# Vigilans/GomokuAI

Measured on AMD Instinct MI355X. Metric: board-evals/s, higher is better.
Workload: dtype int32; 1 GPU; batched AC-automaton position eval (K1), 65536 random-opening boards per GPU, 15x15, inputs resident in HBM; boards_per_gpu=65536, parallelism=boards sharded by rank, no collective, launch=hipGraph replay of the K steps

## Files before the change

gomokuai_amd/csrc/eval_kernel.hip:

```cpp
#include <algorithm>
#include <cstdlib>
#include <vector>

#include "capi_common.h"

namespace {

constexpr int kBoardsPerBlock = 16;
constexpr int kGroupBoards = 16;
constexpr int kThreads = 64 * kBoardsPerBlock;
constexpr int kCells = 225;
constexpr int kQueueCap = 448;
constexpr int kMaxBlocksPerCu = 1;

constexpr int kScoreWords = 4 * kCells;
constexpr int kCntWords = 3 * kCells + 1;
constexpr int kZeroWords = kScoreWords + kCntWords;
constexpr int kLineWords = 96;
constexpr int kColBase = 20, kDiagBase = 36, kAntiBase = 65;
#ifndef GMK_K1_TOTALS_COPIES
#define GMK_K1_TOTALS_COPIES 8
#endif
constexpr int kTotalsCopies = GMK_K1_TOTALS_COPIES;
constexpr int kMiscWords = 48;
constexpr int kBoardWords = kZeroWords + kLineWords + kQueueCap + kMiscWords;
static_assert(kZeroWords % 4 == 0 && kBoardWords % 4 == 0, "16-byte alignment of the per-board blocks");
constexpr int kStaticTableWords = 128 + kLineWords + 512 + 1560 + 4;

__constant__ uint32_t c_lane_jobs[64 * 2];
__constant__ uint32_t c_line_init[kLineWords];
constexpr int kScanSteps = 19;

__device__ __forceinline__ int dir_stride(int dir) { return (0x0E100F01u >> (8 * dir)) & 0xFFu; }

__device__ __forceinline__ uint64_t line_symbols(uint32_t line_word, int len) {
    return 2ull | (static_cast<uint64_t>(line_word) << 2) | (0xAull << (2 * len + 2));
}

__device__ __forceinline__ const __attribute__((address_space(3))) uint32_t* lds_word(uint32_t byte_address) {
    return reinterpret_cast<const __attribute__((address_space(3))) uint32_t*>(static_cast<uintptr_t>(byte_address));
}

__device__ __forceinline__ __attribute__((address_space(3))) uint32_t* lds_word_rw(uint32_t byte_address) {
    return reinterpret_cast<__attribute__((address_space(3))) uint32_t*>(static_cast<uintptr_t>(byte_address));
}

__device__ __forceinline__ uint32_t dfa_address(uint32_t table_word, uint32_t four) {
    uint32_t addr;
    asm("v_bfi_b32 %0, %1, %2, %3" : "=v"(addr) : "s"(0x3FF3u), "v"(table_word), "v"(four));
    return addr;
}

__device__ __forceinline__ uint32_t mul24(uint32_t a, uint32_t b) {
    uint32_t r;
    asm("v_mul_u32_u24 %0, %1, %2" : "=v"(r) : "v"(a), "s"(b));
    return r;
}

__device__ __forceinline__ void wave_phase_fence() {
    __builtin_amdgcn_fence(__ATOMIC_RELEASE, "wavefront");
    __builtin_amdgcn_wave_barrier();
    __builtin_amdgcn_fence(__ATOMIC_ACQUIRE, "wavefront");
}

__device__ __forceinline__ void deposit_match(uint32_t w0, uint32_t w1, int cell_at, int dir, int back_step,
                                              uint32_t* s_scores, uint32_t* s_cnt, uint32_t* s_misc, uint32_t* totals ) {
    const int type = w0 & 15, fav = (w0 >> 4) & 1;
    if (type == 8) { atomicOr(&s_misc[1], fav ? 1u : 2u); return; }
    atomicAdd(&totals[type], fav ? 0x10000u : 1u);
    const int endcell = cell_at + static_cast<int>((w0 >> 27) & 1u) * back_step;
    const uint32_t score = dir >= 2 ? (w1 >> 16) : (w1 & 0xFFFFu);
    unsigned long long* pair = reinterpret_cast<unsigned long long*>(s_scores) + fav;
    const uint32_t lo_opp = fav ? score : 0u, hi_opp = fav ? 0u : score;
    const uint32_t tslot = 5u - static_cast<uint32_t>(type);
    const bool feeds = tslot < 3u;
    uint32_t* cnt = s_cnt + (feeds ? tslot : 0u) * kCells;
    const uint32_t one = 1u << (4 * (fav * 4 + dir));
    const int n_dep = (w0 >> 8) & 7;
#pragma unroll
    for (int d = 0; d < 4; ++d) {
        if (d >= n_dep) break;
        const uint32_t f = (w0 >> (11 + 4 * d)) & 15u;
        const int c = endcell + static_cast<int>(f & 7u) * back_step;
        const bool both = (f & 8u) != 0u;
        atomicAdd(&pair[2 * c], (static_cast<unsigned long long>(both ? score : hi_opp) << 32) | (both ? score : lo_opp));
        if (both && feeds) atomicAdd(&cnt[c], one);
    }
}

__device__ __forceinline__ int counter_match(uint32_t w0, int k, int want) {
    const int type = w0 & 15, len = (w0 >> 5) & 7;
    const int back = k - static_cast<int>((w0 >> 27) & 1u) - 6;
    if (!w0 || type != want || back < 0 || back >= len) return -1;
    const int n_dep = (w0 >> 8) & 7;
    bool on_q = false;
#pragma unroll
    for (int d = 0; d < 4; ++d) {
        const uint32_t f = (w0 >> (11 + 4 * d)) & 15u;
        on_q |= d < n_dep && f == (8u | static_cast<uint32_t>(back));
    }
    return on_q ? back : -1;
}

__device__ __forceinline__ void add_counter_cells(uint32_t w0, int back, int q, int stride, uint32_t* opp) {
    const int n_dep = (w0 >> 8) & 7, endcell = q + back * stride;
#pragma unroll
    for (int d = 0; d < 4; ++d) {
        const uint32_t f = (w0 >> (11 + 4 * d)) & 15u;
        if (d < n_dep && static_cast<int>(f & 7u) != back) atomicAdd(&opp[4 * (endcell - static_cast<int>(f & 7u) * stride)], 600u);
    }
}

[[maybe_unused]] constexpr int kDensTiles = 7;
__host__ __device__ constexpr int dens_kt_lo(int m) { return (((32 * m) / 15 - 3) < 0 ? 0 : (32 * m) / 15 - 3) / 2; }
__host__ __device__ constexpr int dens_kt_hi(int m) { return (((32 * m + 31) / 15 + 3) > 14 ? 14 : (32 * m + 31) / 15 + 3) / 2; }
constexpr int kWtabDy = 13, kWtabEntryWords = 4, kWtabKindWords = kWtabDy * 15 * kWtabEntryWords, kWtabWords = 2 * kWtabKindWords;
__host__ __device__ constexpr int block_weight(int dy, int dx) {
    constexpr int w[4][7] = {{1, 3, 4, 0, 4, 3, 1}, {0, 3, 5, 4, 5, 3, 0}, {0, 4, 3, 3, 3, 4, 0}, {2, 0, 0, 1, 0, 0, 2}};
    return w[dy < 0 ? -dy : dy][dx + 3];
}

typedef int v4i __attribute__((ext_vector_type(4)));
typedef int v16i __attribute__((ext_vector_type(16)));

template <int KIND, int M>
__device__ __forceinline__ void density_tile_pass(const uint32_t (&own_rows)[8], const uint32_t (&other_rows)[8], int n_boards, int first_board, int lane,
                                                  const v4i* __restrict__ s_wtab, int32_t* __restrict__ out_density,
                                                  const uint2* __restrict__ s_lut, int plane_stride) {
    constexpr int lo = dens_kt_lo(M), hi = dens_kt_hi(M), nk = hi - lo + 1;
    constexpr int y0 = (32 * M) / 15, y1 = (32 * M + 31) / 15;
    const int n = lane & 31, h = lane >> 5;
    uint32_t occ = 0;
#pragma unroll
    for (int y = y0; y <= y1; ++y) {
        const uint32_t both = own_rows[y / 2] | other_rows[y / 2];
        const uint32_t r = ((y & 1) ? both >> 16 : both) & 0x7FFFu;
        const int at = 15 * y - 32 * M;
        occ |= at >= 0 ? r << at : r >> -at;
    }
    const int cell = 32 * M + n, yo = (cell * 0x8889) >> 19, xo = cell - 15 * yo;
    const v4i* w = s_wtab + KIND * (kWtabKindWords / kWtabEntryWords) + (2 * lo + h - yo + 6) * 15 + xo;
    v16i acc = {0, 0, 0, 0, 0, 0, 0, 0, 0, 0, 0, 0, 0, 0, 0, 0};
#pragma unroll
    for (int k = 0; k < nk; ++k) {
        const uint32_t r = (own_rows[lo + k] >> (16 * h)) & 0x7FFFu;
        const uint2 b0 = s_lut[r & 255u], b1 = s_lut[r >> 8];
        const v4i stones = {static_cast<int>(b0.x), static_cast<int>(b0.y), static_cast<int>(b1.x), static_cast<int>(b1.y)};
        acc = __builtin_amdgcn_mfma_i32_32x32x32_i8(stones, w[30 * k], acc, 0, 0, 0);
    }
    const int n_live = n_boards - first_board;
    int32_t* out = out_density + static_cast<size_t>(first_board) * 4 * plane_stride + KIND * plane_stride + 32 * M + n + h * (2 * 4 * plane_stride);
#pragma unroll
    for (int i = 0; i < 16; i += 2) {
        const int b = 4 * (i / 4) + (i % 4) / 2;
        const uint32_t wd = static_cast<uint32_t>(__builtin_amdgcn_ds_bpermute(8 * b + 16 * h, static_cast<int>(occ)));
        const int neg = __builtin_amdgcn_sbfe(static_cast<int>(wd), n, 1);
        if (b + 2 * h < n_live && plane_stride > 0) {
            out[b * 4 * plane_stride + 1 * 2 * plane_stride] = acc[i] ^ neg;
            out[b * 4 * plane_stride + 0 * 2 * plane_stride] = acc[i + 1] ^ neg;
        }
    }
}

__device__ __forceinline__ void density_planes_out(const uint16_t* __restrict__ planes, int n_boards, int first_board, int lane,
                                                   const v4i* __restrict__ s_wtab, int32_t* __restrict__ out_density,
                                                   const uint2* __restrict__ s_lut, int plane_stride) {
    const int n = lane & 31, plane = n & 1, board = first_board + (n >> 1);
    uint32_t own[8], other[8];
    {
        const uint4* p = reinterpret_cast<const uint4*>(planes + static_cast<size_t>(board < n_boards ? board : first_board) * 32);
        const uint4 a0 = p[plane * 2], a1 = p[plane * 2 + 1], b0 = p[2 - plane * 2], b1 = p[3 - plane * 2];
        own[0] = a0.x; own[1] = a0.y; own[2] = a0.z; own[3] = a0.w; own[4] = a1.x; own[5] = a1.y; own[6] = a1.z; own[7] = a1.w;
        other[0] = b0.x; other[1] = b0.y; other[2] = b0.z; other[3] = b0.w; other[4] = b1.x; other[5] = b1.y; other[6] = b1.z; other[7] = b1.w;
    }
    if ((lane >> 5) == 0 && board < n_boards && plane_stride > 0) {
        uint32_t c224 = 0, w224 = 0;
#pragma unroll
        for (int dy = -3; dy <= 0; ++dy) {
            const int y = 14 + dy;
            const uint32_t r = (y & 1) ? own[y >> 1] >> 16 : own[y >> 1] & 0xFFFFu;
#pragma unroll
            for (int dx = -3; dx <= 0; ++dx) {
                if (block_weight(dy, dx) == 0) continue;
                const uint32_t bit = (r >> (14 + dx)) & 1u;
                c224 += bit;
                w224 += bit * static_cast<uint32_t>(block_weight(dy, dx));
            }
        }
        const uint32_t neg = 0u - (((own[7] | other[7]) >> 14) & 1u);
        int32_t* out = out_density + static_cast<size_t>(board) * 4 * plane_stride + (1 - plane) * 2 * plane_stride;
        out[224] = static_cast<int32_t>(c224 ^ neg);
        out[plane_stride + 224] = static_cast<int32_t>(w224 ^ neg);
    }
#define GMK_PASS(K, M) density_tile_pass<K, M>(own, other, n_boards, first_board, lane, s_wtab, out_density, s_lut, plane_stride); __builtin_amdgcn_sched_barrier(0);
    GMK_PASS(0, 0) GMK_PASS(1, 0) GMK_PASS(0, 1) GMK_PASS(1, 1) GMK_PASS(0, 2) GMK_PASS(1, 2) GMK_PASS(0, 3) GMK_PASS(1, 3)
    GMK_PASS(0, 4) GMK_PASS(1, 4) GMK_PASS(0, 5) GMK_PASS(1, 5) GMK_PASS(0, 6) GMK_PASS(1, 6)
#undef GMK_PASS
}

__global__ __launch_bounds__(kThreads)
void eval_positions_kernel(const uint16_t* __restrict__ planes, int n_boards, int n_groups,
                           int32_t* __restrict__ out_scores, int32_t* __restrict__ out_density,
                           uint32_t* __restrict__ out_totals, int32_t* __restrict__ out_status,
                           const uint32_t* __restrict__ g_trans, const uint32_t* __restrict__ g_records,
                           int trans_words, int record_words, const uint32_t* __restrict__ g_wtab,
                           int phase_mask_arg, unsigned long long* __restrict__ prof) {
#ifdef GMK_PROFILE
    const int phase_mask = phase_mask_arg;
    unsigned long long t_acc[12] = {0, 0, 0, 0, 0, 0, 0, 0, 0, 0, 0, 0}, t_prev = __builtin_amdgcn_s_memtime();
#define GMK_STAMP(k) do { if (prof) { const unsigned long long t_now_ = __builtin_amdgcn_s_memtime(); t_acc[k] += t_now_ - t_prev; t_prev = t_now_; } } while (0)
#else
    constexpr int phase_mask = 0x7F;
    (void)phase_mask_arg; (void)prof;
#define GMK_STAMP(k) do { } while (0)
#endif
    extern __shared__ __attribute__((aligned(16))) uint32_t lds[];
    const uint4* s_rec = reinterpret_cast<const uint4*>(lds + trans_words);
    uint32_t* s_jobs = lds + trans_words + record_words;

    for (int i = threadIdx.x; i < trans_words; i += kThreads) lds[i] = g_trans[i];
    for (int i = threadIdx.x; i < record_words; i += kThreads) lds[trans_words + i] = g_records[i];
    if (threadIdx.x < 128) s_jobs[threadIdx.x] = c_lane_jobs[threadIdx.x];
    uint32_t* s_pads = s_jobs + 128;
    if (threadIdx.x < kLineWords) s_pads[threadIdx.x] = ~c_line_init[threadIdx.x] & 0xAAAAAAAAu;
    uint2* s_lut = reinterpret_cast<uint2*>(s_jobs + 128 + kLineWords);
    if (threadIdx.x < 256) s_lut[threadIdx.x] = make_uint2(((threadIdx.x & 15u) * 0x204081u) & 0x01010101u, ((threadIdx.x >> 4) * 0x204081u) & 0x01010101u);
    uint32_t* s_wtab_words = s_jobs + 128 + kLineWords + 512;
    for (int i = threadIdx.x; i < kWtabWords; i += kThreads) s_wtab_words[i] = g_wtab[i];
    const v4i* s_wtab = reinterpret_cast<const v4i*>(s_wtab_words);
    uint32_t* s_handout = s_wtab_words + kWtabWords;
    if (threadIdx.x < 4) s_handout[threadIdx.x] = threadIdx.x == 0 ? 2u * kBoardsPerBlock : 0u;

    const int wave = __builtin_amdgcn_readfirstlane(threadIdx.x >> 6), lane0 = threadIdx.x & 63;
    uint32_t* s_scores = lds + trans_words + record_words + kStaticTableWords + wave * kBoardWords;
    uint32_t* s_cnt = s_scores + kScoreWords;
    uint32_t* s_lines = s_scores + kZeroWords;
    uint32_t* s_queue = s_lines + kLineWords;
    uint32_t* s_misc = s_queue + kQueueCap;
#ifndef GMK_K1_TOTALS_HOT
    uint32_t* const my_totals = s_queue + kQueueCap - 8 * kTotalsCopies + (lane0 & (kTotalsCopies - 1)) * 8;
#else
    uint32_t* const my_totals = s_misc + 4;
#endif

    GMK_STAMP(0);

    const bool planes_out = out_density != nullptr && (phase_mask & 64) && !(phase_mask & 1024);
    int lane = lane0;
    const uint32_t job_a = c_lane_jobs[lane * 2], job_b = c_lane_jobs[lane * 2 + 1];
    const uint32_t line_init_lo = c_line_init[lane], line_init_hi = c_line_init[min(64 + lane, kLineWords - 1)];
    auto first_bit = [](uint32_t job) -> uint32_t {
        const uint32_t dir = (job >> 5) & 3u, first = (job >> 12) & 255u, y0 = (first * 0x8889u) >> 19, x0 = first - 15u * y0;
        return dir == 2u ? 2u * x0 : dir == 3u ? 2u * y0 : 0u;
    };
    const uint32_t norm_a = first_bit(job_a), norm_b = first_bit(job_b);
    uint32_t* s_rows = s_misc + 16;
    uint32_t cell_row4 = 0, cell_col = 0;
    for (int pass = 0; pass < 4; ++pass) {
        const int c = min(64 * pass + lane, kCells - 1), y = (c * 0x8889) >> 19;
        cell_row4 |= static_cast<uint32_t>(4 * y) << (8 * pass);
        cell_col |= static_cast<uint32_t>(c - 15 * y) << (8 * pass);
    }
    const uint16_t* row_ptr = planes + (lane & 15);
    uint32_t next_black = 0, next_white = 0, cur_black = 0, cur_white = 0;
    auto fetch_row = [&](int b) {
        const uint16_t* p = row_ptr + static_cast<size_t>(min(b, n_boards - 1)) * 32;
        next_black = p[0];
        next_white = p[16];
    };
    auto take_row = [&](int b) -> uint32_t { return lane < 16 && b < n_boards ? cur_black | (cur_white << 16) : 0u; };

    const int wg_g0 = static_cast<int>(static_cast<long long>(n_groups) * blockIdx.x / gridDim.x);
    const int wg_groups = static_cast<int>(static_cast<long long>(n_groups) * (blockIdx.x + 1) / gridDim.x) - wg_g0;
    const int wg_first = wg_g0 * kGroupBoards, wg_boards = min(wg_groups * kGroupBoards, n_boards - wg_first);
    auto hand_out = [&](int which) -> int {
        uint32_t v = 0;
        if (lane0 == 0) v = atomicAdd(&s_handout[which], 1u);
        return __builtin_amdgcn_readfirstlane(static_cast<int>(v));
    };
    int idx = wave, boards_done = 0;
    if (idx < wg_boards) fetch_row(wg_first + idx);
    asm volatile("" : "+v"(next_black), "+v"(next_white));
#pragma unroll 1
    for (;;) {
        const bool live = idx < wg_boards;
        const int board = wg_first + idx;
        cur_black = next_black; cur_white = next_white;
        int idx_next = idx;
        if (live) { idx_next = boards_done == 0 ? kBoardsPerBlock + wave : hand_out(0); fetch_row(wg_first + min(idx_next, wg_boards - 1)); }
        GMK_STAMP(11);

        if (live) {
            {
                uint4* z = reinterpret_cast<uint4*>(s_cnt) + lane;
    #pragma unroll
                for (int i = 0; i < kCntWords / 4; i += 64)
                    if (i + 64 <= kCntWords / 4 || lane < kCntWords / 4 - i) z[i] = make_uint4(0u, 0u, 0u, 0u);
            }
            s_lines[lane] = line_init_lo;
            if (lane < kLineWords - 64) s_lines[64 + lane] = line_init_hi;
            if (lane < kMiscWords) s_misc[lane] = 0;
#ifndef GMK_K1_TOTALS_HOT
            if (lane < 8 * kTotalsCopies) s_queue[kQueueCap - 8 * kTotalsCopies + lane] = 0;
#endif
            const uint32_t my_row = take_row(board);
            wave_phase_fence();
            {
                uint32_t cnt = static_cast<uint32_t>(__popc(my_row & 0x7FFFu)) | (static_cast<uint32_t>(__popc(my_row >> 16)) << 16);
                cnt += static_cast<uint32_t>(__builtin_amdgcn_update_dpp(0, static_cast<int>(cnt), 0x118, 0xF, 0xF, false));
                cnt += static_cast<uint32_t>(__builtin_amdgcn_update_dpp(0, static_cast<int>(cnt), 0x114, 0xF, 0xF, false));
                cnt += static_cast<uint32_t>(__builtin_amdgcn_update_dpp(0, static_cast<int>(cnt), 0x112, 0xF, 0xF, false));
                cnt += static_cast<uint32_t>(__builtin_amdgcn_update_dpp(0, static_cast<int>(cnt), 0x111, 0xF, 0xF, false));
                if (lane == 15) s_misc[0] = cnt;
            }
            {
                const uint32_t r = my_row;
                const uint32_t l1 = (r & 0x3FFF3FFFu) << 1, l2 = (r & 0x1FFF1FFFu) << 2, l3 = (r & 0x0FFF0FFFu) << 3;
                const uint32_t r1 = (r & 0x7FFE7FFEu) >> 1, r2 = (r & 0x7FFC7FFCu) >> 2, r3 = (r & 0x7FF87FF8u) >> 3;
                const int far = static_cast<int>(r | l3 | r3), near = static_cast<int>(r | l1 | l2 | r1 | r2);
                uint32_t g = l1 | l2 | l3 | r1 | r2 | r3;
                g |= static_cast<uint32_t>(__builtin_amdgcn_update_dpp(0, near, 0x111, 0xF, 0xF, true)) | static_cast<uint32_t>(__builtin_amdgcn_update_dpp(0, near, 0x101, 0xF, 0xF, true));
                g |= static_cast<uint32_t>(__builtin_amdgcn_update_dpp(0, near, 0x112, 0xF, 0xF, true)) | static_cast<uint32_t>(__builtin_amdgcn_update_dpp(0, near, 0x102, 0xF, 0xF, true));
                g |= static_cast<uint32_t>(__builtin_amdgcn_update_dpp(0, far, 0x113, 0xF, 0xF, true)) | static_cast<uint32_t>(__builtin_amdgcn_update_dpp(0, far, 0x103, 0xF, 0xF, true));
                const uint32_t empty = ~(r | (r >> 16)) & 0x7FFFu;
                if (lane < 15) s_rows[3 + lane] = r;
                const int gate = static_cast<int>(g & (empty | (empty << 16)));
    #pragma unroll
                for (int pass = 0; pass < 4; ++pass) {
                    const uint32_t gw = static_cast<uint32_t>(__builtin_amdgcn_ds_bpermute(static_cast<int>((cell_row4 >> (8 * pass)) & 0xFFu), gate)) >> ((cell_col >> (8 * pass)) & 0xFFu);
                    if (pass < 3 || lane < kCells - 192)
                        reinterpret_cast<uint4*>(s_scores)[64 * pass + lane] = make_uint4(((gw >> 16) & 1u) * 160u, 0u, 0u, (gw & 1u) * 160u);
                }
            }
            {
                const int y = lane >> 2, part = lane & 3;
                const uint32_t row = __shfl(my_row, min(y, 14));
                uint32_t row_sym = 0;
                for (uint32_t m = lane < 60 ? (row | (row >> 16)) & (0xFu << (4 * part)) & 0x7FFFu : 0u; m; m &= m - 1u) {
                    const int x = __ffs(m) - 1;
                    const uint32_t code = ((row >> x) & 1u) ? 3u : 2u;
                    const uint32_t at_x = code << (2 * x), at_y = code << (2 * y);
                    row_sym |= at_x;
                    atomicXor(&s_lines[kColBase + x], at_y);
                    atomicXor(&s_lines[kDiagBase + x - y + 14], at_x);
                    atomicXor(&s_lines[kAntiBase + x + y], at_y);
                }
                if (row_sym) atomicXor(&s_lines[y], row_sym);
            }
            wave_phase_fence();
            GMK_STAMP(1);
        }
        if (boards_done == 0) __syncthreads();
        if (live) {
            int n_queued = 0;
            if (phase_mask & 2) {
                const int len_a = static_cast<int>(job_a & 31u) - 3, len_b = static_cast<int>(job_b & 31u) - 3;
                uint64_t syms = line_symbols(s_lines[(job_a >> 20) & 127u] >> norm_a, len_a);
                syms |= line_symbols(s_lines[(job_b >> 20) & 127u] >> norm_b, len_b) << (2 * len_a + 6);
                syms |= 0xAAAAAAAAAAAAAAAAull << (2 * (len_a + len_b) + 12);
                const uint32_t cur = static_cast<uint32_t>(syms) << 2;
                const uint32_t rest = static_cast<uint32_t>(syms >> 28);
                uint32_t tw = 0;
                const uint32_t q_base = static_cast<uint32_t>(s_queue - lds) * 4u;
                const uint32_t q_full = q_base + 4u * (kQueueCap - 64);
                uint32_t q_at = q_base;
                auto push = [&](uint32_t word, int step) {
                    const bool emits = word > 0x1FFFFu;
                    const unsigned long long emitters = __ballot(emits);
                    if (emitters) {
                        if (emits) {
                            const uint32_t ahead = __builtin_amdgcn_mbcnt_hi(static_cast<uint32_t>(emitters >> 32), __builtin_amdgcn_mbcnt_lo(static_cast<uint32_t>(emitters), 0u));
                            *lds_word_rw(q_at + 4u * ahead) = (word & ~0x1FFFFu) | (static_cast<uint32_t>(lane) | static_cast<uint32_t>(step) << 6);
                        }
                        q_at = min(q_at + 4u * static_cast<uint32_t>(__popcll(emitters)), q_full);
                    }
                };
#pragma unroll
                for (int step = 0; step < kScanSteps; ++step) {
                    const uint32_t four = step < 15 ? __builtin_amdgcn_ubfe(cur, 2 * step, 4) : __builtin_amdgcn_ubfe(rest, 2 * (step - 15), 4);
                    const uint32_t addr = dfa_address(tw, four);
                    const uint32_t before = tw;
                    tw = *lds_word(addr);
                    if (step > 0) push(before, step - 1);
                }
                push(tw, kScanSteps - 1);
                n_queued = static_cast<int>((q_at - q_base) >> 2);
                if (q_at >= q_full) s_misc[2] = 1;
            }
            wave_phase_fence();
            GMK_STAMP(2);

            if (phase_mask & 4) {
                uint32_t qe_next = s_queue[min(lane, kQueueCap - 1)];
                for (int m = lane; m < n_queued; m += 64) {
                    const uint32_t qe = qe_next;
                    qe_next = s_queue[min(m + 64, kQueueCap - 1)];
                    const int src_lane = qe & 63, src_step = (qe >> 6) & 31;
                    const uint4 rec_now = s_rec[qe >> 17];
                    const uint32_t ja_now = s_jobs[src_lane * 2], jb_now = s_jobs[src_lane * 2 + 1];
                    const int seg_a = ja_now & 31u;
                    const bool second = src_step >= seg_a;
                    const uint32_t job = second ? jb_now : ja_now;
                    const int pos = src_step - 1 - (second ? seg_a : 0);
                    const int dir = (job >> 5) & 3, stride = (job >> 7) & 31;
                    const int cell_at = static_cast<int>((job >> 12) & 255u) + pos * stride;
                    deposit_match(rec_now.x, rec_now.y, cell_at, dir, -stride, s_scores, s_cnt, s_misc, my_totals);
                    if (rec_now.z) deposit_match(rec_now.z, rec_now.w, cell_at, dir, -stride, s_scores, s_cnt, s_misc, my_totals);
                }
            }
            wave_phase_fence();
#ifndef GMK_K1_TOTALS_HOT
            if (lane < 8) {
                const uint32_t* t = s_queue + kQueueCap - 8 * kTotalsCopies + lane;
                uint32_t sum = 0;
#pragma unroll
                for (int c = 0; c < kTotalsCopies; ++c) sum += t[8 * c];
                s_misc[4 + lane] = sum;
            }
#endif
            GMK_STAMP(3);

            int n_cand = 0;
            if (phase_mask & 8) {
                uint32_t any_cnt[4];
    #pragma unroll
                for (int pass = 0; pass < 4; ++pass) {
                    const int qc = min(64 * pass + lane, kCells - 1);
                    any_cnt[pass] = s_cnt[qc] | s_cnt[kCells + qc] | s_cnt[2 * kCells + qc];
                }
    #pragma unroll
                for (int pass = 0; pass < 4; ++pass) {
                    const int q = 64 * pass + lane;
                    const uint32_t any = any_cnt[pass];
                    const uint32_t upper = (any >> 1) | (any >> 2) | (any >> 3);
                    const uint32_t clipped = ((any | upper) & 0x11111111u) + (upper & 0x11111111u);
                    uint32_t cand = mul24(clipped, 0x1111u) & 0xE000u;
                    cand |= mul24(clipped >> 16, 0x11110u) & 0xE0000u;
                    if (pass == 3 && q >= kCells) cand = 0u;
                    const unsigned long long pushers = __ballot(cand != 0u);
                    if (pushers) {
                        if (cand) {
                            const int slot = n_cand + static_cast<int>(__builtin_amdgcn_mbcnt_hi(static_cast<uint32_t>(pushers >> 32),
                                                                       __builtin_amdgcn_mbcnt_lo(static_cast<uint32_t>(pushers), 0u)));
                            if (slot < kQueueCap / 2) s_queue[slot] = static_cast<uint32_t>(q) | cand;
                        }
                        n_cand += __popcll(pushers);
                    }
                }
            }
            wave_phase_fence();
            GMK_STAMP(4);

            if (n_cand > kQueueCap / 2) { s_misc[2] = 1; n_cand = kQueueCap / 2; }
            if (phase_mask & 2048) n_cand = 0;
            int n_comp_q = 0;
            if (phase_mask & 8)
            for (int v0 = 0; v0 < 2 * n_cand; v0 += 64) {
                const int v = v0 + lane;
                const int flag_shift = 13 + 4 * (v & 1);
                const uint32_t ce = s_queue[v >> 1];
                const int q = ce & 255, c = v & 1;
                bool queue = false;
                uint32_t ent1 = 0, ent2 = 0;
                if (v < 2 * n_cand && ((ce >> flag_shift) & 7u)) {
                    const uint32_t f3 = (s_cnt[q] >> (16 * c)) & 0xFFFFu, fd = (s_cnt[kCells + q] >> (16 * c)) & 0xFFFFu, f2 = (s_cnt[2 * kCells + q] >> (16 * c)) & 0xFFFFu;
                    uint32_t dens = 0;
                    const int qy = (q * 0x8889) >> 19, qx = q - 15 * qy;
                    {
                        const int half = c ? 0 : 16;
    #pragma unroll
                        for (int dy = -3; dy <= 3; ++dy) {
                            const uint32_t pattern = dy == 0 ? 0x77u : (dy == 3 || dy == -3) ? 0x49u : 0x3Eu;
                            const uint32_t mask = ((pattern << qx) >> 3) & 0x7FFFu;
                            dens += __popc((s_rows[3 + qy + dy] >> half) & mask);
                        }
                    }
                    if (dens >= 2u) {
                        const uint32_t up3 = (f3 >> 1) | (f3 >> 2) | (f3 >> 3), upd = (fd >> 1) | (fd >> 2) | (fd >> 3), up2 = (f2 >> 1) | (f2 >> 2) | (f2 >> 3);
                        const uint32_t sel3 = (f3 | up3) & 0x1111u;
                        const uint32_t seld = (fd | upd) & 0x1111u & ~sel3;
                        const uint32_t sel2 = (f2 | up2) & 0x1111u & ~(sel3 | seld);
                        const uint32_t strong = sel3 | seld, any_dir = strong | sel2;
                        const uint32_t twice_strong = (sel3 & up3) | (seld & upd), twice = twice_strong | (sel2 & up2);
                        const int n_comp = __popc(any_dir) + __popc(twice), threes = __popc(strong) + __popc(twice_strong);
                        if (n_comp < 2) {
                            s_misc[2] = 1;
                        } else {
                            const int ctype = min(threes, 2);
                            atomicAdd(&s_misc[12 + ctype], c ? 0x10000u : 1u);
                            const uint32_t crit = 600u * static_cast<uint32_t>(n_comp);
                            atomicAdd(reinterpret_cast<unsigned long long*>(s_scores) + 2 * q + c, (static_cast<unsigned long long>(crit) << 32) | crit);
                            queue = n_comp < 3 && !sel3;
                            const uint32_t b1 = static_cast<uint32_t>(__ffs(any_dir) - 1);
                            const uint32_t others = any_dir & (any_dir - 1u);
                            const uint32_t b2 = others ? static_cast<uint32_t>(__ffs(others) - 1) : b1;
                            const uint32_t ux = static_cast<uint32_t>(qx), uy = static_cast<uint32_t>(qy);
                            const uint32_t lines = (static_cast<uint32_t>(kColBase) << 8 | static_cast<uint32_t>(kDiagBase + 14) << 16 | static_cast<uint32_t>(kAntiBase) << 24)
                                                   + ((ux << 8) * 0x10101u) + uy * 0xFF0001u;
                            const uint32_t slots = ux * 0x0101u + uy * 0x1010u;
                            const uint32_t head = static_cast<uint32_t>(q) | (static_cast<uint32_t>(c) << 8);
                            auto entry = [&](uint32_t b) {
                                const uint32_t tslot = ((seld >> b) & 1u) ? 1u : 2u;
                                return head | (b >> 2) << 9 | tslot << 11 | __builtin_amdgcn_ubfe(lines, 2 * b, 8) << 13 | __builtin_amdgcn_ubfe(slots, b, 4) << 20;
                            };
                            ent1 = entry(b1);
                            ent2 = entry(b2);
                        }
                    }
                }
                const unsigned long long queuers = __ballot(queue);
                if (queue) {
                    const uint32_t slot = static_cast<uint32_t>(n_comp_q) + 2u * __builtin_amdgcn_mbcnt_hi(static_cast<uint32_t>(queuers >> 32),
                                                                                                          __builtin_amdgcn_mbcnt_lo(static_cast<uint32_t>(queuers), 0u));
                    if (slot < kQueueCap / 2) { s_queue[kQueueCap / 2 + slot] = ent1; s_queue[kQueueCap / 2 + slot + 1] = ent2; }
                    else s_misc[2] = 1;
                }
                n_comp_q += 2 * __popcll(queuers);
            }
            wave_phase_fence();
            GMK_STAMP(5);

            if (phase_mask & 16) {
                const int n_comp = min(n_comp_q, kQueueCap / 2);
                int lane_4 = lane;
                asm volatile("" : "+v"(lane_4));
                const int grp = lane_4 / 7, kk = lane_4 - 7 * grp, k = 6 + kk, start = k > 7 ? k - 7 : 0;
                for (int m0 = 0; m0 < n_comp; m0 += 9) {
                    const int m = m0 + grp;
                    const bool on = lane < 63 && m < n_comp;
                    const uint32_t ent = on ? s_queue[kQueueCap / 2 + m] : 0u;
                    const int q = ent & 255, c = (ent >> 8) & 1, dir = (ent >> 9) & 3, tslot = (ent >> 11) & 3;
                    const int stride = dir_stride(dir);
                    uint32_t hit_w0 = 0;
                    int hit_back = -1;
                    if (on) {
                        const uint32_t line = (ent >> 13) & 127u;
                        const uint32_t word = s_lines[line] | s_pads[line];
                        const int first = static_cast<int>((ent >> 20) & 15u) + start - 6;
                        const uint32_t cur = __builtin_amdgcn_alignbit(first >= 0 ? 0xAAAAAAAAu : word, first >= 0 ? word : 0xAAAAAAAAu,
                                                                       static_cast<uint32_t>(2 * first) & 31u) << 2;
                        uint32_t tw = 0;
    #pragma unroll
                        for (int i = 0; i < 8; ++i)
                            if (start + i <= k) tw = *lds_word(dfa_address(tw, __builtin_amdgcn_ubfe(cur, 2 * i, 4)));
                        if ((gmk::dev_trans_kinds(tw) >> tslot) & 1u) {
                            const uint4 rec = s_rec[gmk::dev_trans_record(tw)];
                            const int want = 5 - tslot;
                            hit_back = counter_match(rec.x, k, want);
                            hit_w0 = rec.x;
                            if (hit_back < 0) { hit_back = counter_match(rec.z, k, want); hit_w0 = rec.z; }
                        }
                    }
                    const unsigned long long hits = __ballot(hit_back >= 0);
                    const uint32_t mine = static_cast<uint32_t>(hits >> (7 * grp)) & 0x7Fu;
                    if (hit_back >= 0 && (mine & ((1u << kk) - 1u)) == 0u) add_counter_cells(hit_w0, hit_back, q, stride, s_scores + (c ? 2 : 1));
                }
            }
            wave_phase_fence();
            GMK_STAMP(6);

        }

        asm volatile("" : "+v"(next_black), "+v"(next_white));
        GMK_STAMP(7);

        if (planes_out && (!live || (boards_done & 15) == wave)) {
            for (;;) {
                const int burst = hand_out(1);
                if (burst >= wg_groups) break;
                int lane_p = lane0, first_p = (wg_g0 + burst) * kGroupBoards;
                asm volatile("" : "+v"(lane_p), "+s"(first_p));
                density_planes_out(planes, n_boards, first_p, lane_p, s_wtab, out_density, s_lut, (phase_mask & 512) ? 0 : (phase_mask & 256) ? 256 : kCells);
                GMK_STAMP(8);
                if (live) break;
            }
        }
        if (!live) break;
        if (live && (phase_mask & 32)) {
            int lane_b = lane;
            asm volatile("" : "+v"(lane_b));
            if (out_scores) {
                int32_t* dst = out_scores + static_cast<size_t>(board) * kScoreWords + lane_b;
                const int4* src = reinterpret_cast<const int4*>(s_scores);
                const int4 v0 = src[lane_b], v1 = src[lane_b + 64], v2 = src[lane_b + 128], v3 = src[min(lane_b + 192, kCells - 1)];
#ifdef GMK_K1_PLAIN_SCORES
#define GMK_STORE(p, v) (*(p) = (v))
#else
#define GMK_STORE(p, v) __builtin_nontemporal_store(v, p)
#endif
                const bool tail = lane_b + 192 < kCells;
                GMK_STORE(dst, v0.x); GMK_STORE(dst + 64, v1.x); GMK_STORE(dst + 128, v2.x); if (tail) GMK_STORE(dst + 192, v3.x);
                GMK_STORE(dst + kCells, v0.y); GMK_STORE(dst + kCells + 64, v1.y); GMK_STORE(dst + kCells + 128, v2.y); if (tail) GMK_STORE(dst + kCells + 192, v3.y);
                GMK_STORE(dst + 2 * kCells, v0.z); GMK_STORE(dst + 2 * kCells + 64, v1.z); GMK_STORE(dst + 2 * kCells + 128, v2.z); if (tail) GMK_STORE(dst + 2 * kCells + 192, v3.z);
                GMK_STORE(dst + 3 * kCells, v0.w); GMK_STORE(dst + 3 * kCells + 64, v1.w); GMK_STORE(dst + 3 * kCells + 128, v2.w); if (tail) GMK_STORE(dst + 3 * kCells + 192, v3.w);
#undef GMK_STORE
            }
            if (out_totals && lane_b < 11) out_totals[static_cast<size_t>(board) * 11 + lane_b] = s_misc[4 + lane_b];
            if (out_status && lane_b == 0) {
                const uint32_t wbits = s_misc[1], stones = s_misc[0];
                const int stones_b = stones & 0xFFFFu, stones_w = stones >> 16;
                const int winner = (wbits & 1u) ? 1 : (wbits & 2u) ? -1 : 0;
                const bool over = winner != 0 || stones_b + stones_w == kCells;
                const int to_move = over ? 0 : (stones_b == stones_w ? 1 : -1);
                out_status[board] = (over ? 1 : 0) | ((s_misc[2] || phase_mask != 0x7F) ? 2 : 0) | ((winner & 0xFF) << 8) | ((to_move & 0xFF) << 16);
            }
        }
        wave_phase_fence();
        GMK_STAMP(9);
        idx = idx_next; ++boards_done;
    }
#ifdef GMK_PROFILE
    if (prof && lane0 == 0) {
        for (int k = 0; k < 12; ++k) atomicAdd(&prof[k], t_acc[k]);
        atomicAdd(&prof[15], 1ull);
    }
#endif
#undef GMK_STAMP
}

struct LineJob { int len, x0, y0, dir; };

int upload_lane_jobs() {
    std::vector<LineJob> lines;
    for (int i = 0; i < 15; ++i) lines.push_back({15, 0, i, 0});
    for (int i = 0; i < 15; ++i) lines.push_back({15, i, 0, 1});
    for (int d = -10; d <= 10; ++d) lines.push_back({15 - std::abs(d), d > 0 ? d : 0, d > 0 ? 0 : -d, 2});
    for (int k = 4; k <= 24; ++k) { const int x0 = std::min(k, 14); lines.push_back({std::min(k, 28 - k) + 1, x0, k - x0, 3}); }
    std::stable_sort(lines.begin(), lines.end(), [](const LineJob& a, const LineJob& b) { return a.len > b.len; });
    uint32_t jobs[128];
    for (uint32_t& j : jobs) j = 3u | (15u << 20);
    auto pack = [](const LineJob& l) {
        const int line = l.dir == 0 ? l.y0 : l.dir == 1 ? kColBase + l.x0 : l.dir == 2 ? kDiagBase + l.x0 - l.y0 + 14 : kAntiBase + l.x0 + l.y0;
        const int stride = l.dir == 0 ? 1 : l.dir == 1 ? 15 : l.dir == 2 ? 16 : 14;
        return static_cast<uint32_t>((l.len + 3) | (l.dir << 5) | (stride << 7) | ((l.y0 * 15 + l.x0) << 12) | (line << 20));
    };
    int steps = 0;
    for (int lane = 0; lane < 64; ++lane) {
        jobs[lane * 2] = pack(lines[lane]);
        int total = lines[lane].len + 3;
        const int extra = 64 + (63 - lane);
        if (extra < static_cast<int>(lines.size())) { jobs[lane * 2 + 1] = pack(lines[extra]); total += lines[extra].len + 3; }
        steps = std::max(steps, total);
    }
    uint32_t init[kLineWords] = {};
    for (int i = 0; i < 15; ++i) init[i] = init[kColBase + i] = 0x3FFFFFFFu;
    for (int d = 0; d <= 28; ++d) init[kDiagBase + d] = init[kAntiBase + d] = ((1u << (2 * (15 - std::abs(d - 14)))) - 1u) << (2 * std::max(0, d - 14));
    GMK_HIP_CHECK(hipMemcpyToSymbol(HIP_SYMBOL(c_line_init), init, sizeof init));
    GMK_HIP_CHECK(hipMemcpyToSymbol(HIP_SYMBOL(c_lane_jobs), jobs, sizeof jobs));
    if (steps != kScanSteps) { gmk::set_error("lane jobs: %d scan steps, the kernel is built for %d", steps, kScanSteps); return GMK_ERR_STATE; }
    return GMK_OK;
}

int upload_density_weights(uint32_t** d_out) {
    std::vector<int8_t> t(static_cast<size_t>(kWtabWords) * 4, 0);
    for (int kind = 0; kind < 2; ++kind)
        for (int dy = -3; dy <= 3; ++dy)
            for (int xo = 0; xo < 15; ++xo)
                for (int j = 0; j < 15; ++j) {
                    if (std::abs(j - xo) > 3) continue;
                    const int w = block_weight(dy, j - xo);
                    t[((static_cast<size_t>(kind) * kWtabDy + dy + 6) * 15 + xo) * 16 + j] = static_cast<int8_t>(kind == 0 ? (w != 0) : w);
                }
    for (int cell = 0; cell < 224; ++cell)
        for (int kt = dens_kt_lo(cell / 32); kt <= dens_kt_hi(cell / 32); ++kt)
            for (int h = 0; h < 2; ++h) {
                const int dy = 2 * kt + h - cell / 15;
                if (dy < -6 || dy > 6) { gmk::set_error("density weight table: dy %d of cell %d out of range", dy, cell); return GMK_ERR_STATE; }
            }
    for (int cell = 0; cell < 224; ++cell)
        for (int dy = -3; dy <= 3; ++dy) {
            const int y = cell / 15 + dy, m = cell / 32;
            if (y < 0 || y > 14) continue;
            if (y / 2 < dens_kt_lo(m) || y / 2 > dens_kt_hi(m)) { gmk::set_error("density weight table: row %d of cell %d is not covered", y, cell); return GMK_ERR_STATE; }
        }
    GMK_HIP_CHECK(hipMalloc(d_out, t.size()));
    GMK_HIP_CHECK(hipMemcpy(*d_out, t.data(), t.size(), hipMemcpyHostToDevice));
    return GMK_OK;
}

struct Launch { int grid, n_groups; size_t lds; };

Launch plan_launch(int n, const gmk::DeviceState& st) {
    Launch l;
    l.n_groups = (n + kGroupBoards - 1) / kGroupBoards;
    l.grid = std::max(1, std::min(l.n_groups, st.cu_count * kMaxBlocksPerCu));
    l.lds = static_cast<size_t>(kBoardsPerBlock * kBoardWords + st.n_states * 4 + st.n_records * 4 + kStaticTableWords) * 4;
    return l;
}

bool g_jobs_uploaded = false;
uint32_t* g_wtab = nullptr;
}

extern "C" int gmk_eval_batch(const uint16_t* d_planes, int n, int32_t* d_scores, int32_t* d_density,
                              uint32_t* d_totals, int32_t* d_status, void* stream) {
    gmk::DeviceState& st = gmk::device_state();
    if (!st.ready) { gmk::set_error("gmk_init has not succeeded (no CPU fallback)"); return GMK_ERR_STATE; }
    if (n < 0 || (n > 0 && !d_planes)) { gmk::set_error("gmk_eval_batch: bad arguments"); return GMK_ERR_ARG; }
    if (n == 0) return GMK_OK;
    if (!g_jobs_uploaded) {
        int rc = upload_lane_jobs();
        if (rc != GMK_OK) return rc;
        rc = upload_density_weights(&g_wtab);
        if (rc != GMK_OK) return rc;
        GMK_HIP_CHECK(hipFuncSetAttribute(reinterpret_cast<const void*>(eval_positions_kernel), hipFuncAttributeMaxDynamicSharedMemorySize, 160 * 1024));
        g_jobs_uploaded = true;
    }
    const Launch l = plan_launch(n, st);
    if (l.lds > 160u * 1024u) { gmk::set_error("gmk_eval_batch: tables do not fit in LDS (%zu bytes)", l.lds); return GMK_ERR_CAPACITY; }
    static const int phase_mask = gmk::profile_env("GMK_EVAL_PHASE_MASK") ? std::atoi(gmk::profile_env("GMK_EVAL_PHASE_MASK")) : 0x7F;
    unsigned long long* d_prof = nullptr;
    static const bool stamps = gmk::profile_env("GMK_EVAL_PROFILE") != nullptr;
    if (stamps) {
        GMK_HIP_CHECK(hipMalloc(&d_prof, 16 * sizeof(unsigned long long)));
        GMK_HIP_CHECK(hipMemset(d_prof, 0, 16 * sizeof(unsigned long long)));
    }
    hipLaunchKernelGGL(eval_positions_kernel, dim3(l.grid), dim3(kThreads), l.lds, static_cast<hipStream_t>(stream),
                       d_planes, n, l.n_groups, d_scores, d_density, d_totals, d_status,
                       st.d_trans, st.d_records, st.n_states * 4, st.n_records * 4, g_wtab, phase_mask, d_prof);
    GMK_HIP_CHECK(hipGetLastError());
    if (stamps) {
        unsigned long long h[16];
        GMK_HIP_CHECK(hipDeviceSynchronize());
        GMK_HIP_CHECK(hipMemcpy(h, d_prof, sizeof h, hipMemcpyDeviceToHost));
        (void)hipFree(d_prof);
        const char* names[12] = {"staging", "phase0", "scan", "deposits", "phase3", "phase3b", "rescans", "wait-planes", "phaseD", "phase5", "-", "loop-head"};
        const double boards = static_cast<double>(n), waves = static_cast<double>(h[15] ? h[15] : 1);
        double total = 0;
        for (int k = 0; k < 12; ++k) total += static_cast<double>(h[k]);
        std::fprintf(stderr, "[GMK_EVAL_PROFILE] s_memtime cycles per board (wavefront time; %.0f wavefronts, %.0f cycles each):", waves, total / waves);
        for (int k = 0; k < 12; ++k) if (k != 10) std::fprintf(stderr, " %s %.0f", names[k], static_cast<double>(h[k]) / boards);
        std::fprintf(stderr, "\n");
    }
    return GMK_OK;
}

extern "C" int gmk_eval_launch_info(int n, int* grid, int* block, int* lds_bytes) {
    gmk::DeviceState& st = gmk::device_state();
    if (!st.ready) { gmk::set_error("gmk_init has not succeeded"); return GMK_ERR_STATE; }
    const Launch l = plan_launch(std::max(n, 1), st);
    if (grid) *grid = l.grid;
    if (block) *block = kThreads;
    if (lds_bytes) *lds_bytes = static_cast<int>(l.lds);
    return GMK_OK;
}

extern "C" int gmk_eval_batch_host(const uint16_t* h_planes, int n, int32_t* h_scores, int32_t* h_density,
                                   uint32_t* h_totals, int32_t* h_status) {
    gmk::DeviceState& st = gmk::device_state();
    if (!st.ready) { gmk::set_error("gmk_init has not succeeded (no CPU fallback)"); return GMK_ERR_STATE; }
    if (n < 0 || (n > 0 && !h_planes)) { gmk::set_error("gmk_eval_batch_host: bad arguments"); return GMK_ERR_ARG; }
    if (n == 0) return GMK_OK;
    uint16_t* d_planes = nullptr;
    int32_t *d_scores = nullptr, *d_density = nullptr, *d_status = nullptr;
    uint32_t* d_totals = nullptr;
    const size_t nb = static_cast<size_t>(n);
    int rc = GMK_OK;
    auto cleanup = [&]() { (void)hipFree(d_planes); (void)hipFree(d_scores); (void)hipFree(d_density); (void)hipFree(d_totals); (void)hipFree(d_status); };
#define GMK_TRY(expr) do { if ((expr) != hipSuccess) { gmk::set_error("%s failed", #expr); cleanup(); return GMK_ERR_HIP; } } while (0)
    GMK_TRY(hipMalloc(&d_planes, nb * 64));
    GMK_TRY(hipMalloc(&d_scores, nb * 3600));
    GMK_TRY(hipMalloc(&d_density, nb * 3600));
    GMK_TRY(hipMalloc(&d_totals, nb * 44));
    GMK_TRY(hipMalloc(&d_status, nb * 4));
    GMK_TRY(hipMemcpy(d_planes, h_planes, nb * 64, hipMemcpyHostToDevice));
    rc = gmk_eval_batch(d_planes, n, d_scores, d_density, d_totals, d_status, nullptr);
    if (rc != GMK_OK) { cleanup(); return rc; }
    GMK_TRY(hipDeviceSynchronize());
    if (h_scores) GMK_TRY(hipMemcpy(h_scores, d_scores, nb * 3600, hipMemcpyDeviceToHost));
    if (h_density) GMK_TRY(hipMemcpy(h_density, d_density, nb * 3600, hipMemcpyDeviceToHost));
    if (h_totals) GMK_TRY(hipMemcpy(h_totals, d_totals, nb * 44, hipMemcpyDeviceToHost));
    if (h_status) GMK_TRY(hipMemcpy(h_status, d_status, nb * 4, hipMemcpyDeviceToHost));
#undef GMK_TRY
    cleanup();
    return GMK_OK;
}
```

Before: 524.3 million board-evals/s.

## Precompute occupancy masks in LDS and specialize full-group density stores

The density output pass now computes the per-tile occupancy bitmasks once per group into shared memory (reusing the queue buffer) instead of recomputing them per tile and fetching them with ds_bpermute. Full 16-board groups take a templated path that stores through scalar-base global_store_dword with no per-store bounds checks, while partial groups keep the guarded path. Per-lane row/column and diagonal normalization constants move to a host-computed constant table. This adds LDS reuse of s_queue, which could conflict if that buffer is still live, and relies on inline asm addressing.

```diff
diff --git a/gomokuai_amd/csrc/eval_kernel.hip b/gomokuai_amd/csrc/eval_kernel.hip
--- a/gomokuai_amd/csrc/eval_kernel.hip
+++ b/gomokuai_amd/csrc/eval_kernel.hip
@@ -29,6 +29,7 @@
 
 __constant__ uint32_t c_lane_jobs[64 * 2];
 __constant__ uint32_t c_line_init[kLineWords];
+__constant__ uint4 c_lane_consts[64];
 constexpr int kScanSteps = 19;
 
 __device__ __forceinline__ int dir_stride(int dir) { return (0x0E100F01u >> (8 * dir)) & 0xFFu; }
@@ -55,6 +56,10 @@
     uint32_t r;
     asm("v_mul_u32_u24 %0, %1, %2" : "=v"(r) : "v"(a), "s"(b));
     return r;
+}
+
+__device__ __forceinline__ void store_saddr(uint32_t byte_offset, int32_t value, unsigned long long base) {
+    asm volatile("global_store_dword %0, %1, %2" : : "v"(byte_offset), "v"(value), "s"(base) : "memory");
 }
 
 __device__ __forceinline__ void wave_phase_fence() {
@@ -123,21 +128,14 @@
 typedef int v4i __attribute__((ext_vector_type(4)));
 typedef int v16i __attribute__((ext_vector_type(16)));
 
-template <int KIND, int M>
-__device__ __forceinline__ void density_tile_pass(const uint32_t (&own_rows)[8], const uint32_t (&other_rows)[8], int n_boards, int first_board, int lane,
-                                                  const v4i* __restrict__ s_wtab, int32_t* __restrict__ out_density,
-                                                  const uint2* __restrict__ s_lut, int plane_stride) {
+template <bool kFull, int KIND, int M>
+__device__ __forceinline__ void density_tile_pass(const uint32_t (&own_rows)[8], int n_live, int lane,
+                                                  const v4i* __restrict__ s_wtab, const uint4* __restrict__ s_occ, int32_t* __restrict__ group_out,
+                                                  unsigned long long& board_base , const uint2* __restrict__ s_lut, int plane_stride) {
     constexpr int lo = dens_kt_lo(M), hi = dens_kt_hi(M), nk = hi - lo + 1;
-    constexpr int y0 = (32 * M) / 15, y1 = (32 * M + 31) / 15;
     const int n = lane & 31, h = lane >> 5;
-    uint32_t occ = 0;
-#pragma unroll
-    for (int y = y0; y <= y1; ++y) {
-        const uint32_t both = own_rows[y / 2] | other_rows[y / 2];
-        const uint32_t r = ((y & 1) ? both >> 16 : both) & 0x7FFFu;
-        const int at = 15 * y - 32 * M;
-        occ |= at >= 0 ? r << at : r >> -at;
-    }
+    const uint4 occ_lo = s_occ[4 * M + 2 * h], occ_hi = s_occ[4 * M + 2 * h + 1];
+    const uint32_t occ[8] = {occ_lo.x, occ_lo.y, occ_lo.z, occ_lo.w, occ_hi.x, occ_hi.y, occ_hi.z, occ_hi.w};
     const int cell = 32 * M + n, yo = (cell * 0x8889) >> 19, xo = cell - 15 * yo;
     const v4i* w = s_wtab + KIND * (kWtabKindWords / kWtabEntryWords) + (2 * lo + h - yo + 6) * 15 + xo;
     v16i acc = {0, 0, 0, 0, 0, 0, 0, 0, 0, 0, 0, 0, 0, 0, 0, 0};
@@ -148,32 +146,62 @@
         const v4i stones = {static_cast<int>(b0.x), static_cast<int>(b0.y), static_cast<int>(b1.x), static_cast<int>(b1.y)};
         acc = __builtin_amdgcn_mfma_i32_32x32x32_i8(stones, w[30 * k], acc, 0, 0, 0);
     }
-    const int n_live = n_boards - first_board;
-    int32_t* out = out_density + static_cast<size_t>(first_board) * 4 * plane_stride + KIND * plane_stride + 32 * M + n + h * (2 * 4 * plane_stride);
-#pragma unroll
-    for (int i = 0; i < 16; i += 2) {
-        const int b = 4 * (i / 4) + (i % 4) / 2;
-        const uint32_t wd = static_cast<uint32_t>(__builtin_amdgcn_ds_bpermute(8 * b + 16 * h, static_cast<int>(occ)));
-        const int neg = __builtin_amdgcn_sbfe(static_cast<int>(wd), n, 1);
-        if (b + 2 * h < n_live && plane_stride > 0) {
-            out[b * 4 * plane_stride + 1 * 2 * plane_stride] = acc[i] ^ neg;
-            out[b * 4 * plane_stride + 0 * 2 * plane_stride] = acc[i + 1] ^ neg;
-        }
-    }
-}
-
+    const uint32_t at = static_cast<uint32_t>(KIND * plane_stride + 32 * M + n + h * (2 * 4 * plane_stride));
+    if (kFull) {
+        const uint32_t at_white = 4u * at, at_black = 4u * (at + 2u * static_cast<uint32_t>(plane_stride));
+#pragma unroll
+        for (int i = 0; i < 16; i += 2) {
+            const int neg = __builtin_amdgcn_sbfe(static_cast<int>(occ[i / 2]), n, 1);
+            store_saddr(at_black, acc[i] ^ neg, board_base);
+            store_saddr(at_white, acc[i + 1] ^ neg, board_base);
+            board_base += static_cast<long long>(i == 14 ? -13 : i % 4 ? 3 : 1) * (4 * 4 * plane_stride);
+            asm volatile("" : "+s"(board_base));
+        }
+    } else {
+        int32_t* out = group_out + at;
+#pragma unroll
+        for (int i = 0; i < 16; i += 2) {
+            const int b = 4 * (i / 4) + (i % 4) / 2;
+            const int neg = __builtin_amdgcn_sbfe(static_cast<int>(occ[i / 2]), n, 1);
+            asm volatile("" : "+s"(n_live));
+            if (b + 2 * h < n_live && plane_stride > 0) {
+                out[b * 4 * plane_stride + 1 * 2 * plane_stride] = acc[i] ^ neg;
+                out[b * 4 * plane_stride + 0 * 2 * plane_stride] = acc[i + 1] ^ neg;
+            }
+        }
+    }
+}
+
+template <bool kFull>
 __device__ __forceinline__ void density_planes_out(const uint16_t* __restrict__ planes, int n_boards, int first_board, int lane,
-                                                   const v4i* __restrict__ s_wtab, int32_t* __restrict__ out_density,
+                                                   const v4i* __restrict__ s_wtab, uint32_t* __restrict__ s_occ, int32_t* __restrict__ out_density,
                                                    const uint2* __restrict__ s_lut, int plane_stride) {
     const int n = lane & 31, plane = n & 1, board = first_board + (n >> 1);
     uint32_t own[8], other[8];
     {
-        const uint4* p = reinterpret_cast<const uint4*>(planes + static_cast<size_t>(board < n_boards ? board : first_board) * 32);
+        const uint4* p = reinterpret_cast<const uint4*>(planes + static_cast<size_t>(kFull || board < n_boards ? board : first_board) * 32);
         const uint4 a0 = p[plane * 2], a1 = p[plane * 2 + 1], b0 = p[2 - plane * 2], b1 = p[3 - plane * 2];
         own[0] = a0.x; own[1] = a0.y; own[2] = a0.z; own[3] = a0.w; own[4] = a1.x; own[5] = a1.y; own[6] = a1.z; own[7] = a1.w;
         other[0] = b0.x; other[1] = b0.y; other[2] = b0.z; other[3] = b0.w; other[4] = b1.x; other[5] = b1.y; other[6] = b1.z; other[7] = b1.w;
     }
-    if ((lane >> 5) == 0 && board < n_boards && plane_stride > 0) {
+    if ((lane & 33) == 0) {
+        const int bg = lane >> 1;
+        uint32_t* slot = s_occ + 8 * ((bg >> 1) & 1) + 2 * (bg >> 2) + (bg & 1);
+#pragma unroll
+        for (int m = 0; m < kDensTiles; ++m) {
+            const int y0 = (32 * m) / 15, y1 = (32 * m + 31) / 15;
+            uint32_t occ = 0;
+#pragma unroll
+            for (int y = y0; y <= y1; ++y) {
+                const uint32_t both = own[y / 2] | other[y / 2];
+                const uint32_t r = ((y & 1) ? both >> 16 : both) & 0x7FFFu;
+                const int at = 15 * y - 32 * m;
+                occ |= at >= 0 ? r << at : r >> -at;
+            }
+            slot[16 * m] = occ;
+        }
+    }
+    if ((lane >> 5) == 0 && (kFull || (board < n_boards && plane_stride > 0))) {
         uint32_t c224 = 0, w224 = 0;
 #pragma unroll
         for (int dy = -3; dy <= 0; ++dy) {
@@ -192,7 +220,14 @@
         out[224] = static_cast<int32_t>(c224 ^ neg);
         out[plane_stride + 224] = static_cast<int32_t>(w224 ^ neg);
     }
-#define GMK_PASS(K, M) density_tile_pass<K, M>(own, other, n_boards, first_board, lane, s_wtab, out_density, s_lut, plane_stride); __builtin_amdgcn_sched_barrier(0);
+    const int n_live = __builtin_amdgcn_readfirstlane(n_boards - first_board);
+    int32_t* group_out = out_density + static_cast<size_t>(first_board) * 4 * plane_stride;
+    const uint4* occ_words = reinterpret_cast<const uint4*>(s_occ);
+    const unsigned long long group_bits = reinterpret_cast<unsigned long long>(group_out);
+    unsigned long long board_base = static_cast<unsigned long long>(static_cast<uint32_t>(__builtin_amdgcn_readfirstlane(static_cast<int>(group_bits >> 32)))) << 32
+                                    | static_cast<uint32_t>(__builtin_amdgcn_readfirstlane(static_cast<int>(group_bits)));
+    asm volatile("" : "+s"(board_base));
+#define GMK_PASS(K, M) density_tile_pass<kFull, K, M>(own, n_live, lane, s_wtab, occ_words, group_out, board_base, s_lut, plane_stride); __builtin_amdgcn_sched_barrier(0);
     GMK_PASS(0, 0) GMK_PASS(1, 0) GMK_PASS(0, 1) GMK_PASS(1, 1) GMK_PASS(0, 2) GMK_PASS(1, 2) GMK_PASS(0, 3) GMK_PASS(1, 3)
     GMK_PASS(0, 4) GMK_PASS(1, 4) GMK_PASS(0, 5) GMK_PASS(1, 5) GMK_PASS(0, 6) GMK_PASS(1, 6)
 #undef GMK_PASS
@@ -249,18 +284,9 @@
     int lane = lane0;
     const uint32_t job_a = c_lane_jobs[lane * 2], job_b = c_lane_jobs[lane * 2 + 1];
     const uint32_t line_init_lo = c_line_init[lane], line_init_hi = c_line_init[min(64 + lane, kLineWords - 1)];
-    auto first_bit = [](uint32_t job) -> uint32_t {
-        const uint32_t dir = (job >> 5) & 3u, first = (job >> 12) & 255u, y0 = (first * 0x8889u) >> 19, x0 = first - 15u * y0;
-        return dir == 2u ? 2u * x0 : dir == 3u ? 2u * y0 : 0u;
-    };
-    const uint32_t norm_a = first_bit(job_a), norm_b = first_bit(job_b);
+    const uint4 lane_consts = c_lane_consts[lane];
+    const uint32_t cell_row4 = lane_consts.x, cell_col = lane_consts.y, norm_a = lane_consts.z, norm_b = lane_consts.w;
     uint32_t* s_rows = s_misc + 16;
-    uint32_t cell_row4 = 0, cell_col = 0;
-    for (int pass = 0; pass < 4; ++pass) {
-        const int c = min(64 * pass + lane, kCells - 1), y = (c * 0x8889) >> 19;
-        cell_row4 |= static_cast<uint32_t>(4 * y) << (8 * pass);
-        cell_col |= static_cast<uint32_t>(c - 15 * y) << (8 * pass);
-    }
     const uint16_t* row_ptr = planes + (lane & 15);
     uint32_t next_black = 0, next_white = 0, cur_black = 0, cur_white = 0;
     auto fetch_row = [&](int b) {
@@ -570,7 +596,9 @@
                 if (burst >= wg_groups) break;
                 int lane_p = lane0, first_p = (wg_g0 + burst) * kGroupBoards;
                 asm volatile("" : "+v"(lane_p), "+s"(first_p));
-                density_planes_out(planes, n_boards, first_p, lane_p, s_wtab, out_density, s_lut, (phase_mask & 512) ? 0 : (phase_mask & 256) ? 256 : kCells);
+                const int plane_stride = (phase_mask & 512) ? 0 : (phase_mask & 256) ? 256 : kCells;
+                if (first_p + kGroupBoards <= n_boards && plane_stride > 0) density_planes_out<true>(planes, n_boards, first_p, lane_p, s_wtab, s_queue, out_density, s_lut, plane_stride);
+                else density_planes_out<false>(planes, n_boards, first_p, lane_p, s_wtab, s_queue, out_density, s_lut, plane_stride);
                 GMK_STAMP(8);
                 if (live) break;
             }
@@ -645,6 +673,22 @@
     uint32_t init[kLineWords] = {};
     for (int i = 0; i < 15; ++i) init[i] = init[kColBase + i] = 0x3FFFFFFFu;
     for (int d = 0; d <= 28; ++d) init[kDiagBase + d] = init[kAntiBase + d] = ((1u << (2 * (15 - std::abs(d - 14)))) - 1u) << (2 * std::max(0, d - 14));
+    uint32_t consts[64][4];
+    for (int lane = 0; lane < 64; ++lane) {
+        uint32_t row4 = 0, col = 0;
+        for (int pass = 0; pass < 4; ++pass) {
+            const int c = std::min(64 * pass + lane, kCells - 1);
+            row4 |= static_cast<uint32_t>(4 * (c / 15)) << (8 * pass);
+            col |= static_cast<uint32_t>(c % 15) << (8 * pass);
+        }
+        consts[lane][0] = row4;
+        consts[lane][1] = col;
+        for (int k = 0; k < 2; ++k) {
+            const uint32_t job = jobs[lane * 2 + k], dir = (job >> 5) & 3u, first = (job >> 12) & 255u;
+            consts[lane][2 + k] = dir == 2u ? 2u * (first % 15u) : dir == 3u ? 2u * (first / 15u) : 0u;
+        }
+    }
+    GMK_HIP_CHECK(hipMemcpyToSymbol(HIP_SYMBOL(c_lane_consts), consts, sizeof consts));
     GMK_HIP_CHECK(hipMemcpyToSymbol(HIP_SYMBOL(c_line_init), init, sizeof init));
     GMK_HIP_CHECK(hipMemcpyToSymbol(HIP_SYMBOL(c_lane_jobs), jobs, sizeof jobs));
     if (steps != kScanSteps) { gmk::set_error("lane jobs: %d scan steps, the kernel is built for %d", steps, kScanSteps); return GMK_ERR_STATE; }
```

New measurement: 549.3 million board-evals/s (median of 6 runs). +4.8%, better.
